# nhcha6/embodied-object-detection

Hardware: AMD Instinct MI355X
Metric: frames/sec (640x640, implicit_memory); frames/sec/GPU = value / n_gpus (higher is better)
Workload: dtype f32

## Files before the change

embodied_object_detection_amd/build.py:

```python
from __future__ import annotations

import os
import subprocess
import sys

HERE = os.path.dirname(os.path.abspath(__file__))
CSRC = os.path.join(HERE, "csrc")
LIB = os.path.join(HERE, "libeod_hip.so")
SOURCES = ["conv_igemm.hip", "conv_fp32.hip", "conv_bf16x3.hip", "conv_f16.hip", "elementwise.hip", "roi_align.hip", "select.hip", "heads.hip", "memory.hip", "memory_read.hip", "memory_backward.hip", "conv_wgrad.hip", "train_losses.hip"]
ARCH = "gfx950"


def _stale() -> bool:
    if not os.path.exists(LIB):
        return True
    t = os.path.getmtime(LIB)
    deps = [os.path.join(CSRC, f) for f in os.listdir(CSRC)] + [os.path.join(HERE, "..", "include", "eod_hip.h")]
    return any(os.path.getmtime(d) > t for d in deps if os.path.exists(d))


def _usage_file(src: str) -> str:
    return os.path.join(HERE, "build", src.replace(".hip", ".usage.txt"))


def resource_usage() -> dict:
    import re
    out = {}
    for src in SOURCES:
        f = _usage_file(src)
        if not os.path.exists(f):
            continue
        cur = None
        for line in open(f):
            m = re.search(r"Function Name: (\S+)", line)
            if m:
                cur = out.setdefault(m.group(1), {})
                continue
            for key, pat in (("vgprs", r"\bVGPRs: (\d+)"), ("scratch", r"ScratchSize \[bytes/lane\]: (\d+)"),
                             ("occupancy", r"Occupancy \[waves/SIMD\]: (\d+)"), ("lds", r"LDS Size \[bytes/block\]: (\d+)")):
                m = re.search(pat, line)
                if m and cur is not None:
                    cur[key] = int(m.group(1))
    return out


def scratch_offenders(usage: dict = None) -> list:
    usage = resource_usage() if usage is None else usage
    return sorted(k for k, v in usage.items() if v.get("scratch", 0) > 0)


def build(force: bool = False, verbose: bool = True) -> str:
    if not force and not _stale():
        return LIB
    hipcc = os.environ.get("HIPCC", "/opt/rocm/bin/hipcc")
    objs = []
    procs = []
    os.makedirs(os.path.join(HERE, "build"), exist_ok=True)
    for src in SOURCES:
        obj = os.path.join(HERE, "build", src.replace(".hip", ".o"))
        cmd = [hipcc, f"--offload-arch={ARCH}", "-O3", "-fPIC", "-std=c++17", "-Wall", "-Wno-unused-function",
               "-ffp-contract=on", "-Rpass-analysis=kernel-resource-usage", "-c", os.path.join(CSRC, src), "-o", obj]
        if verbose:
            print(" ".join(cmd), flush=True)
        procs.append((src, subprocess.Popen(cmd, stderr=open(_usage_file(src), "w"))))
        objs.append(obj)
    failed = [s for s, p in procs if p.wait() != 0]
    for src in SOURCES:
        skip = 0
        for line in open(_usage_file(src)):
            if "kernel-resource-usage" in line:
                skip = 2 if "Function Name" in line else 0
                continue
            if skip and (line.lstrip()[:1].isdigit() or line.strip().startswith("|")):
                skip -= 1
                continue
            skip = 0
            if line.strip():
                sys.stderr.write(line)
    if failed:
        raise RuntimeError(f"hipcc failed for {failed}")
    bad = scratch_offenders()
    if bad:
        raise RuntimeError("kernels that use scratch memory (register spills / an argument struct copied to private memory): " + ", ".join(bad))
    cmd = [hipcc, f"--offload-arch={ARCH}", "-shared", "-fPIC", "-o", LIB] + objs
    if verbose:
        print(" ".join(cmd), flush=True)
    subprocess.check_call(cmd)
    return LIB


if __name__ == "__main__":
    build(force="--force" in sys.argv)
    print(LIB)
```

embodied_object_detection_amd/csrc/conv_common.h:

```cpp
#pragma once
#include "eod_common.h"
#include "../../include/eod_hip.h"

namespace eodconv {


struct ConvArgs {
  const float* x;
  const float* w;
  const float* bias;
  const float* res;
  const float* gate;
  float* y;
  float* partial;
  const int* m_count;
  int m_unit;
  int m_segs, seg_rows;
  const float* fuse_w;
  const int* out_units;
  float fuse_b;
  int N, H, W, Cin, OH, OW, Cout, KH, KW, stride, pad, Kpad;
  int M, nchunks, splitk, cps;
  int relu, res_mode, in_relu, out_mode;
  int tiles_m, tiles_n;
  float out_scale;
  int nlv;
  int lv_off[EOD_MAX_LEVELS + 1], lv_h[EOD_MAX_LEVELS], lv_w[EOD_MAX_LEVELS];
  unsigned x_bytes, w_bytes;
  const void* w3;
  unsigned w3_bytes;
  const void* wh;
  unsigned wh_bytes;
  double* gn_partial;
  int gn_groups;
  float* y2;
  int split_n;
  FastDiv div_ow, div_oh, div_cd, div_row;
};

__device__ __forceinline__ int conv_row_limit(const ConvArgs& p, int M) {
  if (p.m_count && p.m_segs <= 1) {
    const int lim = *p.m_count * p.m_unit;
    M = lim < M ? lim : M;
  }
  return M;
}

__device__ __forceinline__ bool conv_row_active(const ConvArgs& p, int m) {
  if (!p.m_count || p.m_segs <= 1) return true;
  const int s = m / p.seg_rows;
  return m - s * p.seg_rows < p.m_count[s] * p.m_unit;
}

__device__ __forceinline__ bool conv_tile_active(const ConvArgs& p, int m0, int bm) {
  if (!p.m_count || p.m_segs <= 1) return true;
  const int last = (m0 + bm - 1 < p.M ? m0 + bm - 1 : p.M - 1);
  const int s0 = m0 / p.seg_rows, s1 = last / p.seg_rows;
  if (m0 - s0 * p.seg_rows < p.m_count[s0] * p.m_unit) return true;
  for (int s = s0 + 1; s <= s1; ++s)
    if (p.m_count[s] > 0) return true;
  return false;
}

template <bool GATE = false>
__device__ __forceinline__ float epilogue_store(const ConvArgs& p, float v, int m, int n) {
  int co = n;
  size_t oidx;
  if (p.out_mode == 1) {
    const int Cd = p.Cout >> 2;
    const int quad = (int)fdiv((unsigned)n, p.div_cd);
    co = n - quad * Cd;
    const int dy = quad >> 1, dx = quad & 1;
    const int t = (int)fdiv((unsigned)m, p.div_ow);
    const int ox = m - t * p.OW;
    const int img = (int)fdiv((unsigned)t, p.div_oh);
    const int oy = t - img * p.OH;
    oidx = ((size_t)(img * 2 * p.OH + 2 * oy + dy) * (2 * p.OW) + (2 * ox + dx)) * Cd + co;
  } else {
    oidx = (size_t)m * p.Cout + n;
  }
  if (p.bias) v += p.bias[co];
  v *= p.out_scale;
  if (p.res_mode == 1) {
    v += p.res[(size_t)m * p.Cout + n];
  } else if (p.res_mode == 2) {
    const int t = (int)fdiv((unsigned)m, p.div_ow);
    const int ox = m - t * p.OW;
    const int img = (int)fdiv((unsigned)t, p.div_oh);
    const int oy = t - img * p.OH;
    const int rh = p.OH >> 1, rw = p.OW >> 1;
    v += p.res[((size_t)(img * rh + (oy >> 1)) * rw + (ox >> 1)) * p.Cout + n];
  }
  if (p.split_n > 0) {
    if (n >= p.split_n) {
      if (p.relu) v = fmaxf(v, 0.0f);
      p.y2[(size_t)m * (p.Cout - p.split_n) + (n - p.split_n)] = v;
    } else {
      p.y[(size_t)m * p.split_n + n] = v;
    }
    return v;
  }
  if (p.relu) v = fmaxf(v, 0.0f);
  if (GATE && p.gate && !(p.gate[oidx] > 0.0f)) v = 0.0f;
  p.y[oidx] = v;
  return v;
}

__device__ __forceinline__ unsigned long long tap_mask(int iy0, int ix0, int hh, int ww, int KH, int KW) {
  unsigned long long mask = 0;
  int tp = 0;
  for (int ky = 0; ky < KH; ++ky) {
    const bool rok = (unsigned)(iy0 + ky) < (unsigned)hh;
    for (int kx = 0; kx < KW; ++kx, ++tp) {
      const bool ok = rok && ((unsigned)(ix0 + kx) < (unsigned)ww);
      mask |= (unsigned long long)ok << tp;
    }
  }
  return mask;
}

template <int TM, int TN, bool GATE = false>
__device__ __forceinline__ void store_wave_tiles(const ConvArgs& p, const f32x16 (&acc)[TM][TN], int m_base, int n_base, int M, int z,
                                                 int lane) {
  const int half = lane >> 5;
#pragma unroll
  for (int i = 0; i < TM; ++i) {
#pragma unroll
    for (int j = 0; j < TN; ++j) {
      const int n = n_base + j * 32 + (lane & 31);
#pragma unroll
      for (int r = 0; r < 16; ++r) {
        const int row = (r & 3) + 8 * (r >> 2) + 4 * half;
        const int m = m_base + i * 32 + row;
        if (m < M && n < p.Cout && conv_row_active(p, m)) {
          const float v = acc[i][j][r];
          if (p.splitk > 1) {
            p.partial[((size_t)z * p.M + m) * p.Cout + n] = v;
          } else {
            epilogue_store<GATE>(p, v, m, n);
          }
        }
      }
    }
  }
}

void launch_conv_fp32(const ConvArgs& a, int tile, int bk, bool tap4, dim3 grid, hipStream_t s, int lds_reserve = 0, int prefetch2 = 0);
void launch_conv_bf16x3(const ConvArgs& a, int tile, dim3 grid, hipStream_t s);
void launch_conv_wavek(const ConvArgs& a, int nw, dim3 grid, hipStream_t s);
void launch_split_weights(const float* w, void* out, int Cout, int Kpad, hipStream_t s);
void launch_conv_f16(const ConvArgs& a, int tile, int bk, dim3 grid, hipStream_t s);
void launch_half_weights(const float* w, void* out, int Cout, int Kpad, hipStream_t s);

}
```

embodied_object_detection_amd/csrc/conv_igemm.hip:

```cpp
#include "conv_common.h"
#include "../../include/eod_hip.h"
#include <atomic>
#include <cstdlib>
#include <cstring>

namespace {

using namespace eodconv;

template <int VEC>
__global__ __launch_bounds__(256) void conv_splitk_reduce_kernel(ConvArgs p) {
  EOD_CHAIN_PRIO();
  const int M = conv_row_limit(p, p.M);
  const unsigned per_row = (unsigned)p.Cout / VEC;
  const unsigned total = (unsigned)M * per_row;
  const size_t slab = (size_t)p.M * p.Cout;
  for (unsigned idx = blockIdx.x * blockDim.x + threadIdx.x; idx < total; idx += gridDim.x * blockDim.x) {
    const unsigned m = fdiv(idx, p.div_row);
    if (!conv_row_active(p, (int)m)) continue;
    const unsigned n = (idx - m * per_row) * VEC;
    const float* src = p.partial + (size_t)m * p.Cout + n;
    if (VEC == 4) {
      f32x4 v = {0.f, 0.f, 0.f, 0.f};
      for (int zb = 0; zb < p.splitk; zb += 4) {
        f32x4 t[4];
#pragma unroll
        for (int j = 0; j < 4; ++j)
          if (zb + j < p.splitk) t[j] = *reinterpret_cast<const f32x4*>(src + (size_t)(zb + j) * slab);
#pragma unroll
        for (int j = 0; j < 4; ++j)
          if (zb + j < p.splitk) v += t[j];
      }
      epilogue_store<true>(p, v.x, (int)m, (int)n);
      epilogue_store<true>(p, v.y, (int)m, (int)n + 1);
      epilogue_store<true>(p, v.z, (int)m, (int)n + 2);
      epilogue_store<true>(p, v.w, (int)m, (int)n + 3);
    } else {
      float v = 0.f;
      for (int z = 0; z < p.splitk; ++z) v += src[z * slab];
      epilogue_store<true>(p, v, (int)m, (int)n);
    }
  }
}

#define EOD_GN_ROWS 32
__global__ __launch_bounds__(256) void conv_splitk_reduce_gn_kernel(ConvArgs p) {
  EOD_CHAIN_PRIO();
  __shared__ double red[4][64][2];
  int level = 0, first_chunk = 0;
  for (;;) {
    const int rows = p.lv_off[level + 1] - p.lv_off[level];
    const int nch = (rows + EOD_GN_ROWS - 1) / EOD_GN_ROWS;
    if ((int)blockIdx.x < first_chunk + nch || level + 1 >= p.nlv) break;
    first_chunk += nch;
    ++level;
  }
  const int r0 = p.lv_off[level] + ((int)blockIdx.x - first_chunk) * EOD_GN_ROWS;
  const int r1 = min(r0 + EOD_GN_ROWS, p.lv_off[level + 1]);
  const int C = p.Cout;
  const int c4 = C >> 2;
  const int nsub = 256 / c4;
  const int col = threadIdx.x % c4, sub = threadIdx.x / c4;
  const int cpg4 = (C / p.gn_groups) >> 2;
  const size_t slab = (size_t)p.M * C;
  double s = 0.0, q = 0.0;
  for (int r = r0 + sub; r < r1; r += nsub) {
    const float* src = p.partial + (size_t)r * C + col * 4;
    f32x4 v = {0.f, 0.f, 0.f, 0.f};
    for (int zb = 0; zb < p.splitk; zb += 4) {
      f32x4 t[4];
#pragma unroll
      for (int j = 0; j < 4; ++j)
        if (zb + j < p.splitk) t[j] = *reinterpret_cast<const f32x4*>(src + (size_t)(zb + j) * slab);
#pragma unroll
      for (int j = 0; j < 4; ++j)
        if (zb + j < p.splitk) v += t[j];
    }
    const double o0 = (double)epilogue_store<true>(p, v.x, r, col * 4 + 0);
    const double o1 = (double)epilogue_store<true>(p, v.y, r, col * 4 + 1);
    const double o2 = (double)epilogue_store<true>(p, v.z, r, col * 4 + 2);
    const double o3 = (double)epilogue_store<true>(p, v.w, r, col * 4 + 3);
    s += o0; q += o0 * o0;
    s += o1; q += o1 * o1;
    s += o2; q += o2 * o2;
    s += o3; q += o3 * o3;
  }
  for (int off = 1; off < cpg4; off <<= 1) {
    s += __shfl_xor(s, off, 64);
    q += __shfl_xor(q, off, 64);
  }
  if ((col % cpg4) == 0) {
    red[sub][col / cpg4][0] = s;
    red[sub][col / cpg4][1] = q;
  }
  __syncthreads();
  if ((int)threadIdx.x < p.gn_groups) {
    double ts = 0.0, tq = 0.0;
    for (int u = 0; u < nsub; ++u) {
      ts += red[u][threadIdx.x][0];
      tq += red[u][threadIdx.x][1];
    }
    p.gn_partial[((size_t)blockIdx.x * p.gn_groups + threadIdx.x) * 2 + 0] = ts;
    p.gn_partial[((size_t)blockIdx.x * p.gn_groups + threadIdx.x) * 2 + 1] = tq;
  }
}

std::atomic<int>& math_mode() {
  static std::atomic<int> v([] {
    const char* e = getenv("EOD_CONV_MATH");
    if (e && strcmp(e, "bf16x3") == 0) return EOD_MATH_BF16X3;
    if (e && strcmp(e, "f16") == 0) return EOD_MATH_F16;
    return EOD_MATH_FP32;
  }());
  return v;
}

struct Plan {
  int tile;
  int bk;
  int glds;
  int bm, bn, tiles_m, tiles_n, splitk, cps, nchunks;
  int wavek;
};

Plan make_plan(const EodConvDesc* d, int M) {
  static const int cfg[5][2] = {{128, 128}, {128, 64}, {64, 64}, {256, 128}, {64, 256}};
  Plan pl{};
  int pick = 2;
  const int ft = d->force_tile % 10, fbk = d->force_tile / 10;
  const bool half_ok = !d->tap4 && !d->in_relu;
  const bool f16_forced = (fbk == 8 || fbk == 9) && half_ok;
  if (f16_forced) pick = ft == 4 ? 3 : 2;
  else if (ft >= 1 && ft <= 3) pick = ft - 1;
  else if (ft == 4 && fbk == 5 && half_ok) pick = 3;
  const bool bk64_ok = !d->tap4 && d->Cin % 64 == 0 && d->Kpad % 64 == 0;
  pl.glds = f16_forced ? 3 : ((fbk == 5 && half_ok) ? 2 : 0);
  const int Mp = (d->plan_rows > 0 && d->plan_rows < M) ? d->plan_rows : M;
  const int math = d->math > 0 ? d->math - 1 : math_mode().load(std::memory_order_relaxed);
  if (d->force_tile == 0 && math == EOD_MATH_F16 && half_ok) {
    pl.glds = 3;
    pick = (long)((Mp + 255) / 256) * ((d->Cout + 127) / 128) >= 256 ? 3 : 2;
  }
  if (d->force_tile == 0 && math == EOD_MATH_BF16X3 && half_ok) {
    pl.glds = 2;
    const long t128 = (long)((Mp + 127) / 128) * ((d->Cout + 127) / 128);
    const long t256 = (long)((Mp + 255) / 256) * ((d->Cout + 127) / 128);
    pick = t256 >= 256 ? 3 : (t128 >= 512 ? 0 : 2);
  }
  if (d->out_mode == 2) {
    pick = 4;
    pl.glds = 0;
  }
  if (d->gate) {
    const bool f16_gated = d->math == EOD_MATH_F16 + 1 && half_ok && d->levels <= 0 && (d->force_tile == 0 || f16_forced);
    pick = 2;
    pl.glds = f16_gated ? 3 : 0;
  }
  if (pl.glds == 3) pl.bk = (fbk == 8 && d->Cin % 64 == 0) ? 64 : 32;
  else pl.bk = (pl.glds == 0 && d->out_mode != 2 && fbk == 2 && bk64_ok) ? 64 : 32;
  const int nchunks = d->Kpad / pl.bk;
  pl.nchunks = nchunks;
  pl.tile = pick + 1;
  pl.bm = cfg[pick][0];
  pl.bn = cfg[pick][1];
  pl.tiles_m = (M + pl.bm - 1) / pl.bm;
  pl.tiles_n = (d->Cout + pl.bn - 1) / pl.bn;
  const long tiles = (long)((Mp + pl.bm - 1) / pl.bm) * pl.tiles_n;
  int splitk = 1;
  if (d->out_mode == 2) {
    splitk = 1;
  } else if (d->force_splitk > 0) {
    splitk = d->force_splitk;
  } else if (pl.glds == 0 && !d->tap4 && nchunks >= 8 &&
             ((d->force_tile == 6 || d->force_tile == 7) ||
              (tiles < 256 && nchunks <= 192 && pl.bk == 32 && d->force_tile == 0 &&
               ((Mp <= 512 && nchunks / (nchunks >= 64 ? 8 : 4) >= 8) || nchunks >= 128)))) {
    pl.wavek = d->force_tile == 6 ? 4 : (d->force_tile == 7 ? 8 : (nchunks >= 64 ? 8 : 4));
    pl.bk = 32;
    pl.nchunks = d->Kpad / 32;
    pl.bm = pl.bn = 32;
    pl.tiles_m = (M + 31) / 32;
    pl.tiles_n = (d->Cout + 31) / 32;
  } else if (tiles < 256 && nchunks >= 8) {
    const int target = (nchunks >= 128 && Mp <= 512) ? 1792 : 512;
    int want = (int)((target + tiles - 1) / tiles);
    int maxs = nchunks / 4;
    splitk = want < maxs ? want : maxs;
    if (splitk < 1) splitk = 1;
  } else if (tiles >= 256 && tiles <= 1024 && d->m_count == nullptr && nchunks >= 18) {
    double best = 1e30;
    for (int sct = 1; sct <= 4; ++sct) {
      if (nchunks / sct < 9) break;
      const double est = (double)((tiles * sct + 255) / 256) / sct + (sct > 1 ? 0.12 : 0.0);
      if (est < best - 1e-9) {
        best = est;
        splitk = sct;
      }
    }
  }
  if (splitk > nchunks) splitk = nchunks;
  pl.cps = (nchunks + splitk - 1) / splitk;
  pl.splitk = (nchunks + pl.cps - 1) / pl.cps;
  return pl;
}

int total_rows(const EodConvDesc* d) { return d->levels > 0 ? d->level_off[d->levels] : d->N * d->OH * d->OW; }

int check_desc(const EodConvDesc* d) {
  if (!d || !d->x || !d->w || !d->y) return EOD_ERR_NULL;
  if (d->N <= 0 || d->Cin <= 0 || d->Cout <= 0) return EOD_ERR_BAD_DIMS;
  if (d->levels <= 0 && (d->H <= 0 || d->W <= 0 || d->OH <= 0 || d->OW <= 0)) return EOD_ERR_BAD_DIMS;
  if (d->KH <= 0 || d->KW <= 0 || d->stride <= 0 || d->pad < 0) return EOD_ERR_BAD_DIMS;
  if (d->Kpad % 32 != 0 || d->Kpad < d->KH * d->KW * d->Cin) return EOD_ERR_BAD_DIMS;
  if (d->tap4) {
    if (d->Cin != 4) return EOD_ERR_BAD_DIMS;
  } else {
    if (d->Cin % 32 != 0 || d->Kpad != d->KH * d->KW * d->Cin) return EOD_ERR_BAD_DIMS;
  }
  if (d->levels > 0) {
    if (d->levels > EOD_MAX_LEVELS || d->N != 1 || d->stride != 1 || d->KH != d->KW || d->pad != d->KH / 2 || d->tap4 || d->out_mode != 0 ||
        d->res_mode == 2 || d->level_off[0] != 0)
      return EOD_ERR_BAD_DIMS;
    for (int l = 0; l < d->levels; ++l)
      if (d->level_h[l] <= 0 || d->level_w[l] <= 0 || d->level_off[l + 1] - d->level_off[l] != d->level_h[l] * d->level_w[l])
        return EOD_ERR_BAD_DIMS;
  } else {
    if (d->OH != (d->H + 2 * d->pad - d->KH) / d->stride + 1) return EOD_ERR_BAD_DIMS;
    if (d->OW != (d->W + 2 * d->pad - d->KW) / d->stride + 1) return EOD_ERR_BAD_DIMS;
  }
  if (d->levels <= 0 && (long)d->N * d->H * d->W * d->Cin >= (1L << 29)) return EOD_ERR_BAD_DIMS;
  if ((long)d->Cout * d->Kpad >= (1L << 29)) return EOD_ERR_BAD_DIMS;
  if (d->KH * d->KW > 64) return EOD_ERR_BAD_DIMS;
  if ((long)total_rows(d) * (d->Cout > d->Cin ? d->Cout : d->Cin) >= (1L << 31)) return EOD_ERR_BAD_DIMS;
  if (d->out_mode == 1 && (d->Cout % 4 != 0)) return EOD_ERR_BAD_DIMS;
  if (d->out_mode == 2) {
    if (d->Cout != 1024 || d->KH != 1 || d->KW != 1 || d->stride != 1 || d->tap4 || d->levels > 0 || d->res_mode != 0 || d->in_relu ||
        d->force_splitk > 1)
      return EOD_ERR_BAD_DIMS;
    if (!d->fuse_w) return EOD_ERR_NULL;
  }
  if (d->out_mode < 0 || d->out_mode > 2) return EOD_ERR_BAD_DIMS;
  if (d->res_mode != 0 && !d->res) return EOD_ERR_NULL;
  if (d->res_mode == 2 && ((d->OH & 1) || (d->OW & 1))) return EOD_ERR_BAD_DIMS;
  if (d->m_count && d->m_unit <= 0) return EOD_ERR_BAD_DIMS;
  if (d->m_segments > 1) {
    if (!d->m_count || d->levels > 0 || d->out_mode == 2 || d->m_segments > EOD_MAX_BATCH || d->N % d->m_segments != 0)
      return EOD_ERR_BAD_DIMS;
    if (((long)(d->N / d->m_segments) * d->OH * d->OW) % d->m_unit != 0) return EOD_ERR_BAD_DIMS;
  }
  if (d->gate && (d->out_mode != 0 || d->split_n != 0 || d->gn_partial)) return EOD_ERR_BAD_DIMS;
  if (d->gate && d->force_tile != 0 && d->force_tile % 10 != 3 && d->force_tile != 6 && d->force_tile != 7) return EOD_ERR_BAD_DIMS;
  if (d->gate && d->force_tile / 10 == 5) return EOD_ERR_BAD_DIMS;
  if (d->gate && (d->force_tile / 10 == 8 || d->force_tile / 10 == 9) &&
      (d->math != EOD_MATH_F16 + 1 || d->force_tile % 10 != 3 || d->levels > 0 || d->tap4 || d->in_relu))
    return EOD_ERR_BAD_DIMS;
  if (d->math < 0 || d->math > EOD_MATH_F16 + 1) return EOD_ERR_BAD_DIMS;
  if ((d->force_tile / 10 == 8 || d->force_tile / 10 == 9) && d->force_tile % 10 != 3 && d->force_tile % 10 != 4) return EOD_ERR_BAD_DIMS;
  if (d->lds_reserve < 0 || d->lds_reserve > 48 * 1024) return EOD_ERR_BAD_DIMS;
  if (d->split_n != 0) {
    if (!d->y2) return EOD_ERR_NULL;
    if (d->split_n < 0 || d->split_n >= d->Cout || d->out_mode != 0 || d->res_mode != 0 || d->levels > 0 || d->gn_partial)
      return EOD_ERR_BAD_DIMS;
  }
  if (d->gn_partial) {
    const int cpg = d->gn_groups > 0 ? d->Cout / d->gn_groups : 0;
    if (d->levels <= 0 || d->m_count || d->out_mode != 0 || d->gn_groups <= 0 || d->gn_groups > 64 || d->Cout % d->gn_groups != 0 ||
        cpg > 64 || (cpg & (cpg - 1)) != 0 || cpg < 4 || d->Cout % 4 != 0 || d->Cout > 1024 || 256 % (d->Cout / 4) != 0 ||
        64 % (cpg / 4) != 0)
      return EOD_ERR_BAD_DIMS;
  }
  if (!eod_aligned16(d->x) || !eod_aligned16(d->w) || !eod_aligned16(d->w_split) || !eod_aligned16(d->w_half)) return EOD_ERR_ALIGN;
  return EOD_OK;
}

}

extern "C" int eod_set_conv_math(int mode) {
  if (mode != EOD_MATH_FP32 && mode != EOD_MATH_BF16X3 && mode != EOD_MATH_F16) return EOD_ERR_BAD_DIMS;
  return math_mode().exchange(mode);
}

extern "C" int eod_get_conv_math(void) { return math_mode().load(); }

extern "C" size_t eod_conv_split_weights_bytes(int Cout, int Kpad) {
  return (Cout > 0 && Kpad > 0 && Kpad % 32 == 0) ? (size_t)Cout * Kpad * 6 : 0;
}

extern "C" int eod_conv_split_weights_bf16x3(const float* w, int Cout, int Kpad, void* out, eod_stream_t stream) {
  if (!w || !out) return EOD_ERR_NULL;
  if (Cout <= 0 || Kpad <= 0 || Kpad % 32 != 0 || (long)Cout * Kpad * 6 >= (1L << 32)) return EOD_ERR_BAD_DIMS;
  if (!eod_aligned16(w) || !eod_aligned16(out)) return EOD_ERR_ALIGN;
  launch_split_weights(w, out, Cout, Kpad, static_cast<hipStream_t>(stream));
  return eod_launch_status();
}

extern "C" size_t eod_conv_half_weights_bytes(int Cout, int Kpad) {
  return (Cout > 0 && Kpad > 0 && Kpad % 32 == 0) ? (size_t)Cout * Kpad * 2 : 0;
}

extern "C" int eod_conv_half_weights(const float* w, int Cout, int Kpad, void* out, eod_stream_t stream) {
  if (!w || !out) return EOD_ERR_NULL;
  if (Cout <= 0 || Kpad <= 0 || Kpad % 32 != 0 || (long)Cout * Kpad >= (1L << 29)) return EOD_ERR_BAD_DIMS;
  if (!eod_aligned16(w) || !eod_aligned16(out)) return EOD_ERR_ALIGN;
  launch_half_weights(w, out, Cout, Kpad, static_cast<hipStream_t>(stream));
  return eod_launch_status();
}

extern "C" int eod_conv2d_gn_fused(const EodConvDesc* d) {
  EodConvDesc t = *d;
  t.gn_partial = nullptr;
  if (check_desc(&t) != EOD_OK) return 0;
  return make_plan(&t, total_rows(&t)).splitk > 1 ? 1 : 0;
}

extern "C" int eod_conv2d_plan(const EodConvDesc* d, EodConvPlan* out) {
  if (!out) return EOD_ERR_NULL;
  const int st = check_desc(d);
  if (st != EOD_OK) return st;
  const Plan pl = make_plan(d, total_rows(d));
  out->tile = pl.tile; out->bm = pl.bm; out->bn = pl.bn; out->bk = pl.bk;
  out->splitk = pl.splitk; out->cps = pl.cps; out->nchunks = pl.nchunks;
  out->wavek = pl.wavek; out->glds = pl.glds;
  out->tiles_m = pl.tiles_m; out->tiles_n = pl.tiles_n;
  out->gn_fused = (d->gn_partial && pl.splitk > 1) ? 1 : 0;
  return EOD_OK;
}

extern "C" size_t eod_conv2d_workspace_bytes(const EodConvDesc* d) {
  if (check_desc(d) != EOD_OK) return 0;
  const int M = total_rows(d);
  const Plan pl = make_plan(d, M);
  if (pl.splitk <= 1) return 0;
  return (size_t)pl.splitk * M * d->Cout * sizeof(float);
}

extern "C" int eod_conv2d(const EodConvDesc* d, eod_stream_t stream) {
  const int st = check_desc(d);
  if (st != EOD_OK) return st;
  hipStream_t s = static_cast<hipStream_t>(stream);
  ConvArgs a{};
  a.x = d->x; a.w = d->w; a.bias = d->bias; a.res = d->res; a.y = d->y;
  a.partial = d->workspace;
  a.m_count = d->m_count; a.m_unit = d->m_unit;
  a.m_segs = d->m_segments > 1 ? d->m_segments : 1;
  a.seg_rows = a.m_segs > 1 ? (d->N / d->m_segments) * d->OH * d->OW : 0;
  a.fuse_w = d->fuse_w; a.out_units = d->out_units; a.fuse_b = d->fuse_b;
  a.N = d->N; a.H = d->H; a.W = d->W; a.Cin = d->Cin; a.OH = d->OH; a.OW = d->OW; a.Cout = d->Cout;
  a.KH = d->KH; a.KW = d->KW; a.stride = d->stride; a.pad = d->pad; a.Kpad = d->Kpad;
  a.M = total_rows(d);
  a.div_ow = eod_make_fastdiv((unsigned)(d->OW > 0 ? d->OW : 1));
  a.div_oh = eod_make_fastdiv((unsigned)(d->OH > 0 ? d->OH : 1));
  a.div_row = eod_make_fastdiv((unsigned)(d->Cout % 4 == 0 ? d->Cout / 4 : d->Cout));
  a.div_cd = eod_make_fastdiv((unsigned)((d->Cout >> 2) > 0 ? (d->Cout >> 2) : 1));
  {
    const size_t xe = d->levels > 0 ? (size_t)d->level_off[d->levels] * d->Cin : (size_t)d->N * d->H * d->W * d->Cin;
    a.x_bytes = (unsigned)(xe * sizeof(float));
    a.w_bytes = (unsigned)((size_t)d->Cout * d->Kpad * sizeof(float));
    a.w3 = d->w_split;
    a.w3_bytes = (unsigned)((size_t)d->Cout * d->Kpad * 6);
    a.wh = d->w_half;
    a.wh_bytes = (unsigned)((size_t)d->Cout * d->Kpad * 2);
  }
  a.nlv = d->levels > 0 ? d->levels : 0;
  for (int l = 0; l < a.nlv; ++l) {
    a.lv_off[l] = d->level_off[l];
    a.lv_h[l] = d->level_h[l];
    a.lv_w[l] = d->level_w[l];
  }
  if (a.nlv) a.lv_off[a.nlv] = d->level_off[a.nlv];
  a.relu = d->relu; a.res_mode = d->res_mode; a.in_relu = d->in_relu; a.out_mode = d->out_mode;
  a.gate = d->gate;
  a.out_scale = d->out_scale;
  a.gn_partial = d->gn_partial;
  a.gn_groups = d->gn_groups;
  a.y2 = d->y2;
  a.split_n = d->split_n;
  const Plan pl = make_plan(d, a.M);
  if (d->gn_partial && pl.splitk <= 1) return EOD_ERR_BAD_DIMS;
  a.nchunks = pl.nchunks;
  a.splitk = pl.splitk; a.cps = pl.cps; a.tiles_m = pl.tiles_m; a.tiles_n = pl.tiles_n;
  if (pl.splitk > 1) {
    const size_t need = (size_t)pl.splitk * a.M * a.Cout * sizeof(float);
    if (!d->workspace || d->workspace_bytes < need) return EOD_ERR_CAPACITY;
  }
  dim3 grid(pl.tiles_m * pl.tiles_n, pl.splitk);
  if (pl.wavek) launch_conv_wavek(a, pl.wavek, grid, s);
  else if (pl.glds == 3) launch_conv_f16(a, pl.tile, pl.bk, grid, s);
  else if (pl.glds == 2) launch_conv_bf16x3(a, pl.tile, grid, s);
  else launch_conv_fp32(a, pl.tile, pl.bk, d->tap4 != 0, grid, s, d->lds_reserve, d->prefetch2);
  if (pl.splitk > 1) {
    const size_t total = (size_t)a.M * a.Cout;
    const bool vec = a.Cout % 4 == 0;
    int blocks = (int)((total / (vec ? 4 : 1) + 255) / 256);
    if (blocks > 2048) blocks = 2048;
    if (blocks < 1) blocks = 1;
    if (a.gn_partial) {
      int chunks = 0;
      for (int l = 0; l < a.nlv; ++l) chunks += (a.lv_off[l + 1] - a.lv_off[l] + EOD_GN_ROWS - 1) / EOD_GN_ROWS;
      hipLaunchKernelGGL(conv_splitk_reduce_gn_kernel, dim3(chunks), dim3(256), 0, s, a);
    } else if (vec) hipLaunchKernelGGL(conv_splitk_reduce_kernel<4>, dim3(blocks), dim3(256), 0, s, a);
    else hipLaunchKernelGGL(conv_splitk_reduce_kernel<1>, dim3(blocks), dim3(256), 0, s, a);
  }
  return eod_launch_status();
}
```

Measured before the change: 298.7.

## Add dedicated FP32 MFMA kernel for 1x1 pointwise convolutions

Adds a specialised kernel for 1x1 stride-1 FP32 convolutions with Cin of 64/128/256. It keeps the whole 64-row activation tile resident in LDS and streams weights through several 64-column output panels per workgroup with double buffering. Bias and residual loads are prefetched for the next panel. The goal is to reuse activations across output panels instead of reloading them per tile. In exchange it adds a planner path that is auto-selected only for large grids, plus more LDS per workgroup and lower occupancy.

```diff
diff --git a/embodied_object_detection_amd/build.py b/embodied_object_detection_amd/build.py
--- a/embodied_object_detection_amd/build.py
+++ b/embodied_object_detection_amd/build.py
@@ -7,7 +7,7 @@
 HERE = os.path.dirname(os.path.abspath(__file__))
 CSRC = os.path.join(HERE, "csrc")
 LIB = os.path.join(HERE, "libeod_hip.so")
-SOURCES = ["conv_igemm.hip", "conv_fp32.hip", "conv_bf16x3.hip", "conv_f16.hip", "elementwise.hip", "roi_align.hip", "select.hip", "heads.hip", "memory.hip", "memory_read.hip", "memory_backward.hip", "conv_wgrad.hip", "train_losses.hip"]
+SOURCES = ["conv_igemm.hip", "conv_fp32.hip", "conv_pointwise.hip", "conv_bf16x3.hip", "conv_f16.hip", "elementwise.hip", "roi_align.hip", "select.hip", "heads.hip", "memory.hip", "memory_read.hip", "memory_backward.hip", "conv_wgrad.hip", "train_losses.hip"]
 ARCH = "gfx950"
 
 
diff --git a/embodied_object_detection_amd/csrc/conv_common.h b/embodied_object_detection_amd/csrc/conv_common.h
--- a/embodied_object_detection_amd/csrc/conv_common.h
+++ b/embodied_object_detection_amd/csrc/conv_common.h
@@ -148,6 +148,7 @@
 void launch_conv_fp32(const ConvArgs& a, int tile, int bk, bool tap4, dim3 grid, hipStream_t s, int lds_reserve = 0, int prefetch2 = 0);
 void launch_conv_bf16x3(const ConvArgs& a, int tile, dim3 grid, hipStream_t s);
 void launch_conv_wavek(const ConvArgs& a, int nw, dim3 grid, hipStream_t s);
+void launch_conv_pointwise(const ConvArgs& a, int np, dim3 grid, hipStream_t s);
 void launch_split_weights(const float* w, void* out, int Cout, int Kpad, hipStream_t s);
 void launch_conv_f16(const ConvArgs& a, int tile, int bk, dim3 grid, hipStream_t s);
 void launch_half_weights(const float* w, void* out, int Cout, int Kpad, hipStream_t s);
diff --git a/embodied_object_detection_amd/csrc/conv_igemm.hip b/embodied_object_detection_amd/csrc/conv_igemm.hip
--- a/embodied_object_detection_amd/csrc/conv_igemm.hip
+++ b/embodied_object_detection_amd/csrc/conv_igemm.hip
@@ -121,7 +121,19 @@
   int glds;
   int bm, bn, tiles_m, tiles_n, splitk, cps, nchunks;
   int wavek;
+  int pw_np;
 };
+
+constexpr int kForcePointwise = 30;
+
+int effective_math(const EodConvDesc* d) { return d->math > 0 ? d->math - 1 : math_mode().load(std::memory_order_relaxed); }
+
+bool pointwise_eligible(const EodConvDesc* d) {
+  return effective_math(d) == EOD_MATH_FP32 && d->KH == 1 && d->KW == 1 && d->stride == 1 && d->pad == 0 && d->levels <= 0 && !d->tap4 &&
+         d->Cin == d->Kpad && (d->Cin == 64 || d->Cin == 128 || d->Cin == 256) && d->Cout % 64 == 0 && d->out_mode == 0 &&
+         (d->res_mode == 0 || d->res_mode == 1) && !d->in_relu && !d->gate && !d->m_count && d->split_n == 0 && !d->gn_partial &&
+         d->lds_reserve == 0;
+}
 
 Plan make_plan(const EodConvDesc* d, int M) {
   static const int cfg[5][2] = {{128, 128}, {128, 64}, {64, 64}, {256, 128}, {64, 256}};
@@ -136,7 +148,7 @@
   const bool bk64_ok = !d->tap4 && d->Cin % 64 == 0 && d->Kpad % 64 == 0;
   pl.glds = f16_forced ? 3 : ((fbk == 5 && half_ok) ? 2 : 0);
   const int Mp = (d->plan_rows > 0 && d->plan_rows < M) ? d->plan_rows : M;
-  const int math = d->math > 0 ? d->math - 1 : math_mode().load(std::memory_order_relaxed);
+  const int math = effective_math(d);
   if (d->force_tile == 0 && math == EOD_MATH_F16 && half_ok) {
     pl.glds = 3;
     pick = (long)((Mp + 255) / 256) * ((d->Cout + 127) / 128) >= 256 ? 3 : 2;
@@ -201,6 +213,32 @@
   if (splitk > nchunks) splitk = nchunks;
   pl.cps = (nchunks + splitk - 1) / splitk;
   pl.splitk = (nchunks + pl.cps - 1) / pl.cps;
+  const bool pw_forced = d->force_tile == kForcePointwise && d->force_splitk <= 1;
+  const bool pw_auto = d->force_tile == 0 && d->force_splitk == 0 && pointwise_eligible(d) && pl.splitk == 1 && !pl.wavek && tiles >= 256 &&
+                       !(d->Kpad == 256 && d->Cout < 1024);
+  if (pw_forced || pw_auto) {
+    const int panels = d->Cout / 64;
+    const long row_tiles = (Mp + 63) / 64;
+    const long want = tiles >= 256 ? 512 : 1;
+    int np = 1;
+    for (int cand = 4; cand > 1; cand >>= 1)
+      if (panels >= cand && row_tiles * ((panels + cand - 1) / cand) >= want) {
+        np = cand;
+        break;
+      }
+    pl.pw_np = np;
+    pl.tile = 6;
+    pl.glds = 0;
+    pl.bk = 32;
+    pl.nchunks = d->Kpad / 32;
+    pl.bm = 64;
+    pl.bn = 64 * np;
+    pl.tiles_m = (M + 63) / 64;
+    pl.tiles_n = (panels + np - 1) / np;
+    pl.splitk = 1;
+    pl.cps = pl.nchunks;
+    pl.wavek = 0;
+  }
   return pl;
 }
 
@@ -257,6 +295,7 @@
   if (d->math < 0 || d->math > EOD_MATH_F16 + 1) return EOD_ERR_BAD_DIMS;
   if ((d->force_tile / 10 == 8 || d->force_tile / 10 == 9) && d->force_tile % 10 != 3 && d->force_tile % 10 != 4) return EOD_ERR_BAD_DIMS;
   if (d->lds_reserve < 0 || d->lds_reserve > 48 * 1024) return EOD_ERR_BAD_DIMS;
+  if (d->force_tile == kForcePointwise && (!pointwise_eligible(d) || d->force_splitk > 1)) return EOD_ERR_BAD_DIMS;
   if (d->split_n != 0) {
     if (!d->y2) return EOD_ERR_NULL;
     if (d->split_n < 0 || d->split_n >= d->Cout || d->out_mode != 0 || d->res_mode != 0 || d->levels > 0 || d->gn_partial)
@@ -384,7 +423,8 @@
     if (!d->workspace || d->workspace_bytes < need) return EOD_ERR_CAPACITY;
   }
   dim3 grid(pl.tiles_m * pl.tiles_n, pl.splitk);
-  if (pl.wavek) launch_conv_wavek(a, pl.wavek, grid, s);
+  if (pl.pw_np) launch_conv_pointwise(a, pl.pw_np, grid, s);
+  else if (pl.wavek) launch_conv_wavek(a, pl.wavek, grid, s);
   else if (pl.glds == 3) launch_conv_f16(a, pl.tile, pl.bk, grid, s);
   else if (pl.glds == 2) launch_conv_bf16x3(a, pl.tile, grid, s);
   else launch_conv_fp32(a, pl.tile, pl.bk, d->tap4 != 0, grid, s, d->lds_reserve, d->prefetch2);
diff --git a/embodied_object_detection_amd/csrc/conv_pointwise.hip b/embodied_object_detection_amd/csrc/conv_pointwise.hip
--- /dev/null
+++ b/embodied_object_detection_amd/csrc/conv_pointwise.hip
@@ -0,0 +1,189 @@
+#include "conv_operands.h"
+
+namespace eodconv {
+namespace {
+
+template <int K>
+struct PointwiseCfg {
+  static constexpr int BKW = K == 256 ? 16 : 32;
+  static constexpr int LSA = K + 4;
+  static constexpr int LSW = BKW + 4;
+  static constexpr int A_FLOATS = 64 * LSA;
+  static constexpr int W_FLOATS = 64 * LSW;
+  static constexpr int LDS_BYTES = (A_FLOATS + 2 * W_FLOATS) * 4;
+  static constexpr int WG_PER_CU = K == 256 ? 2 : 3;
+};
+
+template <int K>
+__global__ __launch_bounds__(256) __attribute__((amdgpu_waves_per_eu(PointwiseCfg<K>::WG_PER_CU))) void conv_pointwise_kernel(ConvArgs p, int np) {
+  using Cfg = PointwiseCfg<K>;
+  constexpr int BKW = Cfg::BKW, LSA = Cfg::LSA, LSW = Cfg::LSW;
+  constexpr int NC = K / BKW;
+  constexpr int KS = BKW / 8;
+  constexpr int QPR = BKW / 4;
+  constexpr int RPP = 256 / QPR;
+  constexpr int BR = 64 / RPP;
+  constexpr int AQ = K / 4;
+  constexpr int AR = K / 16;
+  static_assert(NC % 2 == 0, "stage parity");
+  extern __shared__ __attribute__((aligned(16))) float lds[];
+  float* As = lds;
+  float* Ws = lds + Cfg::A_FLOATS;
+
+  const int tid = threadIdx.x;
+  const int lane = tid & 63;
+  const int wave = tid >> 6;
+  const int wm = wave >> 1, wn = wave & 1;
+
+  int M;
+  const int t = conv_first_tile<64>(p, M);
+  if (t < 0) return;
+  const int tile_m = t / p.tiles_n;
+  const int grp = t - tile_m * p.tiles_n;
+  const int m0 = tile_m * 64;
+  const int panels = p.Cout >> 6;
+  const int p0 = grp * np;
+  const int p1 = p0 + np < panels ? p0 + np : panels;
+
+  const __amdgpu_buffer_rsrc_t rsrc_x = conv_buffer(p.x, p.x_bytes);
+  const __amdgpu_buffer_rsrc_t rsrc_w = conv_buffer(p.w, p.w_bytes);
+
+  const int lr = tid / QPR, lq = tid % QPR;
+  auto load_w = [&](int panel, int c, f32x4 (&wr)[BR]) {
+    if (c >= NC) {
+      c -= NC;
+      ++panel;
+    }
+    if (panel >= p1) return;
+#pragma unroll
+    for (int j = 0; j < BR; ++j)
+      wr[j] = __builtin_bit_cast(f32x4, __builtin_amdgcn_raw_buffer_load_b128(rsrc_w, conv_w_row_offset(p, panel * 64 + lr + RPP * j, lq),
+                                                                              c * BKW * 4, 0));
+  };
+  auto store_w = [&](int buf, const f32x4 (&wr)[BR]) {
+#pragma unroll
+    for (int j = 0; j < BR; ++j) *reinterpret_cast<f32x4*>(Ws + buf * Cfg::W_FLOATS + (lr + RPP * j) * LSW + 4 * lq) = wr[j];
+  };
+
+  const int half = lane >> 5;
+  const int m_base = m0 + wm * 32 + 4 * half;
+  const int n_lane = wn * 32 + (lane & 31);
+  auto load_res = [&](int panel, float (&rr)[16], float& bb) {
+    const int n = panel * 64 + n_lane;
+    if (p.bias) bb = p.bias[n];
+    if (p.res_mode == 1) {
+#pragma unroll
+      for (int r = 0; r < 16; ++r) {
+        const int m = m_base + (r & 3) + 8 * (r >> 2);
+        if (m < M) rr[r] = p.res[(unsigned)(m * p.Cout + n)];
+      }
+    }
+  };
+
+  f32x4 w0[BR], w1[BR];
+  float rcur[16], rnext[16];
+  float bcur = 0.f, bnext = 0.f;
+#pragma unroll
+  for (int r = 0; r < 16; ++r) rcur[r] = rnext[r] = 0.f;
+  {
+    f32x4 ar[AR];
+    const unsigned a_off = (unsigned)(m0 * K + 4 * tid) * 4u;
+#pragma unroll
+    for (int i = 0; i < AR; ++i) ar[i] = __builtin_bit_cast(f32x4, __builtin_amdgcn_raw_buffer_load_b128(rsrc_x, a_off + i * 4096u, 0, 0));
+    load_w(p0, 0, w0);
+    load_w(p0, 1, w1);
+    load_res(p0, rcur, bcur);
+#pragma unroll
+    for (int i = 0; i < AR; ++i) {
+      const int idx = i * 256 + tid;
+      *reinterpret_cast<f32x4*>(As + (idx / AQ) * LSA + 4 * (idx % AQ)) = ar[i];
+    }
+    store_w(0, w0);
+  }
+  __syncthreads();
+
+  const int frag_row = lane & 31;
+  const int frag_k = 4 * half;
+  const float* a_base = As + (wm * 32 + frag_row) * LSA + frag_k;
+  const float* b_base = Ws + (wn * 32 + frag_row) * LSW + frag_k;
+
+  f32x16 acc, acc_b;
+  auto stage = [&](int panel, int c, int buf, f32x4 (&hold)[BR], f32x4 (&fill)[BR]) {
+    load_w(panel, c + 2, fill);
+    const float* ab = a_base + c * BKW;
+    const float* bb = b_base + buf * Cfg::W_FLOATS;
+    f32x4 af[2], bf[2];
+    af[0] = *reinterpret_cast<const f32x4*>(ab);
+    bf[0] = *reinterpret_cast<const f32x4*>(bb);
+#pragma unroll
+    for (int kk = 0; kk < KS; ++kk) {
+      const int cur = kk & 1, nxt = cur ^ 1;
+      if (kk + 1 < KS) {
+        af[nxt] = *reinterpret_cast<const f32x4*>(ab + (kk + 1) * 8);
+        bf[nxt] = *reinterpret_cast<const f32x4*>(bb + (kk + 1) * 8);
+      }
+      __builtin_amdgcn_s_setprio(1);
+#pragma unroll
+      for (int tt = 0; tt < 4; ++tt)
+        if (tt & 1)
+          acc_b = __builtin_amdgcn_mfma_f32_32x32x2f32(af[cur][tt], bf[cur][tt], acc_b, 0, 0, 0);
+        else
+          acc = __builtin_amdgcn_mfma_f32_32x32x2f32(af[cur][tt], bf[cur][tt], acc, 0, 0, 0);
+      __builtin_amdgcn_s_setprio(0);
+    }
+    if (c + 1 < NC || panel + 1 < p1) store_w(buf ^ 1, hold);
+    __syncthreads();
+  };
+
+  for (int panel = p0; panel < p1; ++panel) {
+    if (panel + 1 < p1) load_res(panel + 1, rnext, bnext);
+#pragma unroll
+    for (int r = 0; r < 16; ++r) {
+      acc[r] = 0.f;
+      acc_b[r] = 0.f;
+    }
+    for (int c = 0; c < NC; c += 2) {
+      stage(panel, c, 0, w1, w0);
+      stage(panel, c + 1, 1, w0, w1);
+    }
+#pragma unroll
+    for (int r = 0; r < 16; ++r) acc[r] += acc_b[r];
+    const int n = panel * 64 + n_lane;
+#pragma unroll
+    for (int r = 0; r < 16; ++r) {
+      const int m = m_base + (r & 3) + 8 * (r >> 2);
+      if (m < M) {
+        float v = acc[r];
+        if (p.bias) v += bcur;
+        v *= p.out_scale;
+        if (p.res_mode == 1) v += rcur[r];
+        if (p.relu) v = fmaxf(v, 0.0f);
+        p.y[(unsigned)(m * p.Cout + n)] = v;
+      }
+    }
+#pragma unroll
+    for (int r = 0; r < 16; ++r) rcur[r] = rnext[r];
+    bcur = bnext;
+  }
+}
+
+template <int K>
+void launch_pointwise(const ConvArgs& a, int np, dim3 grid, hipStream_t s) {
+  constexpr int kLds = PointwiseCfg<K>::LDS_BYTES;
+  static const bool attr = kLds <= 65536 || hipFuncSetAttribute(reinterpret_cast<const void*>(&conv_pointwise_kernel<K>),
+                                                                hipFuncAttributeMaxDynamicSharedMemorySize, kLds) == hipSuccess;
+  (void)attr;
+  hipLaunchKernelGGL((conv_pointwise_kernel<K>), grid, dim3(256), kLds, s, a, np);
+}
+
+}
+
+void launch_conv_pointwise(const ConvArgs& a, int np, dim3 grid, hipStream_t s) {
+  switch (a.Kpad) {
+    case 64: launch_pointwise<64>(a, np, grid, s); break;
+    case 128: launch_pointwise<128>(a, np, grid, s); break;
+    default: launch_pointwise<256>(a, np, grid, s); break;
+  }
+}
+
+}
```

After: 304.9, median of 6. +2.1%, better.
